# yuliangguo/OmniFusion

Measured on AMD Instinct MI355X. Metric: panoramas/sec at 512x1024 ERP, N=18 256^2 patches; equi2pers+pers2equi GB/s vs HBM peak, higher is better.
Workload: dtype f16x3 (fp16 hi/lo pairs, fp32 accumulate: fp32-class); 1 GPU; cfg2/cfg4 shard: 8 panoramas/GPU/step, 512x1024 ERP, fov 80, nrows 4 (18 patches); full single-pass spherical_fusion forward (confidence=True) at patch size 128 — the only size the reference network exists at (SURVEY 0.1); random-init weights (seed 42); inputs resident in HBM; resample pair at 18x256^2 reported in roofline_resample; per_gpu_batch=8, global_batch=8, parallelism=image-sharded x1, execution=3 forwards in flight per GPU on 3 streams (spherical_fusion.pipelined)

## Files before the change

### omnifusion_amd/csrc/omni_conv_up2_taps.hip

```cpp
#include <stdint.h>
#include "omni_conv_sh_common.h"

namespace {

struct TapsArgs {
    const void* src;
    const void* wt;
    const float* bias;
    void* dst;
    int M, Hl, Cout, act;
};

constexpr int TAP_BYTES = 32 * 256;

__device__ __forceinline__ void wait_taps_in_flight(int n)
{
    if (n >= 16) wait_vm<16>();
    else if (n == 14) wait_vm<14>();
    else if (n == 12) wait_vm<12>();
    else if (n == 10) wait_vm<10>();
    else if (n == 8) wait_vm<8>();
    else if (n == 6) wait_vm<6>();
    else if (n == 4) wait_vm<4>();
    else if (n == 2) wait_vm<2>();
    else wait_vm<0>();
}

template <int WL, int ROWS, int HALO>
__global__ __launch_bounds__(256, 1) void up2_taps_fused_kernel(TapsArgs a)
{
    static_assert((WL == 32 && ROWS == 8 && HALO == 1) || (WL == 16 && ROWS == 16 && HALO == 0), "bands of 8 rows of 32-wide maps, or whole 16 x 16 maps");
    constexpr int SROWS = ROWS + 2 * HALO, P = SROWS * WL, NF = P / 32, NFW = (NF + 3) / 4;
    constexpr int W_BYTES = 9 * TAP_BYTES, CH_BYTES = P * 128, ROW_BYTES = WL * 128;
    static_assert(P % 32 == 0 && ROWS * WL == 256, "whole fragments; one (column, channel quad) thread per eight rows");
    __shared__ __attribute__((aligned(1024))) unsigned char lds[W_BYTES + 2 * CH_BYTES];
    static_assert(sizeof(lds) <= 160 * 1024, "one block per CU");

    const int t = threadIdx.x, lane = t & 63;
    const int wave = __builtin_amdgcn_readfirstlane(t >> 6);
    const int ntn = a.Cout >> 5, nb = a.Hl / ROWS;
    int bid = blockIdx.x;
    const int tile_n = bid % ntn; bid /= ntn;
    const int band = bid % nb; const int m = bid / nb;
    const int r0 = band * ROWS, col0 = tile_n * 32, sbase = r0 - HALO;
    const int Hl = a.Hl;

    auto frag = [&](int fi) { const int f = wave + 4 * fi; return f < NF ? f : wave + 4; };
    h8v xh[NFW][4], xl[NFW][4];
#pragma unroll
    for (int fi = 0; fi < NFW; ++fi) {
        const int f = frag(fi);
        {
            const int p = f * 32 + (lane & 31), sr = p / WL, cx = p - sr * WL;
            const int row = min(max(sbase + sr, 0), Hl - 1);
            const unsigned char* sp = (const unsigned char*)a.src + ((size_t)(m * Hl + row) * WL + cx) * 256 + (lane >> 5) * 16;
#pragma unroll
            for (int kc = 0; kc < 4; ++kc) {
                xh[fi][kc] = *reinterpret_cast<const h8v*>(sp + (kc >> 1) * 128 + (kc & 1) * 32);
                xl[fi][kc] = *reinterpret_cast<const h8v*>(sp + (kc >> 1) * 128 + 64 + (kc & 1) * 32);
            }
        }
    }
    {
        const rsrc_t rsw = make_rsrc(a.wt, (size_t)9 * a.Cout * 256);
#pragma unroll
        for (int tp = 0; tp < 9; ++tp)
#pragma unroll
            for (int k = 0; k < 2; ++k) {
                const int i = wave + 4 * k, row = 4 * i + (lane >> 4), piece = (lane & 15) ^ (row & 15);
                dma16(rsw, lds + tp * TAP_BYTES + i * 1024, ((tp * a.Cout + col0 + row) * 16 + piece) * 16, 0);
            }
    }
    const int wfo = (lane & 31) * 256 + (((lane >> 5) ^ (lane & 15)) * 16);

    const int quad = t & 7, j = (t >> 3) & (WL - 1);
    const int ib = WL == 32 ? 0 : 8 * (wave >> 1);
    int coff[3];
#pragma unroll
    for (int c = 0; c < 3; ++c) {
        const int col = min(max(j - 1 + c, 0), WL - 1);
        coff[c] = col * 128 + ((quad ^ ((col >> 1) & 3)) * 16);
    }
    float hx[4], lx[4];
    hx[0] = j > 0 ? 0.75f : 0.0f;      lx[0] = j > 0 ? 0.25f : 0.0f;
    hx[1] = j > 0 ? 0.25f : 1.0f;      lx[1] = j > 0 ? 0.75f : 0.0f;
    hx[2] = 0.75f;                     lx[2] = 0.25f;
    hx[3] = j < WL - 1 ? 0.25f : 0.0f; lx[3] = j < WL - 1 ? 0.75f : 0.0f;

    f4v out[8][2][2];
#pragma unroll
    for (int it = 0; it < 8; ++it)
#pragma unroll
        for (int ab = 0; ab < 4; ++ab) out[it][ab >> 1][ab & 1] = (f4v)(0.0f);

    wait_taps_in_flight(16);
    __builtin_amdgcn_s_barrier();
    asm volatile("" ::: "memory");

    auto tap = [&]<int tp>() {
        constexpr int ky = tp / 3, kx = tp - 3 * ky;
        unsigned char* chunk = lds + W_BYTES + (tp & 1) * CH_BYTES;
        {
            const unsigned char* wb = lds + tp * TAP_BYTES;
            h8v wh[4], wl[4];
#pragma unroll
            for (int kc = 0; kc < 4; ++kc) {
                const int K = 8 * (kc >> 1) + 2 * (kc & 1);
                wh[kc] = *reinterpret_cast<const h8v*>(wb + (wfo ^ (K * 16)));
                wl[kc] = *reinterpret_cast<const h8v*>(wb + (wfo ^ ((K + 4) * 16)));
            }
#pragma unroll
            for (int fi = 0; fi < NFW; ++fi) {
                const int f = frag(fi);
                {
                    f16v acc = (f16v)(0.0f), acc1 = (f16v)(0.0f);
#pragma unroll
                    for (int kc = 0; kc < 4; ++kc) {
                        acc  = __builtin_amdgcn_mfma_f32_32x32x16_f16(wh[kc], xh[fi][kc], acc, 0, 0, 0);
                        acc1 = __builtin_amdgcn_mfma_f32_32x32x16_f16(wl[kc], xh[fi][kc], acc1, 0, 0, 0);
                        acc1 = __builtin_amdgcn_mfma_f32_32x32x16_f16(wh[kc], xl[fi][kc], acc1, 0, 0, 0);
                    }
                    const int px = f * 32 + (lane & 31);
                    unsigned char* cp = chunk + px * 128;
                    const int sw = (px >> 1) & 3;
#pragma unroll
                    for (int q = 0; q < 4; ++q) {
                        f4v v;
#pragma unroll
                        for (int e = 0; e < 4; ++e) v[e] = acc_join<false>(acc1[4 * q + e], acc[4 * q + e]);
                        *reinterpret_cast<f4v*>(cp + (((2 * q + (lane >> 5)) ^ sw) * 16)) = v;
                    }
                }
                __builtin_amdgcn_sched_barrier(0);
            }
        }
        if (tp < 8) wait_taps_in_flight(2 * (7 - tp));
        wait_lds_reads();
        __builtin_amdgcn_s_barrier();
        asm volatile("" ::: "memory");
#pragma unroll
        for (int it = 0; it < 8; ++it) {
            const int i = r0 + ib + it;
            float hy[4], ly[4];
            const bool top = it == 0 && i == 0, bot = it == 7 && i == Hl - 1;
            hy[0] = top ? 0.0f : 0.75f; ly[0] = top ? 0.0f : 0.25f;
            hy[1] = top ? 1.0f : 0.25f; ly[1] = top ? 0.0f : 0.75f;
            hy[2] = 0.75f;              ly[2] = 0.25f;
            hy[3] = bot ? 0.0f : 0.25f; ly[3] = bot ? 0.0f : 0.75f;
            f4v v[3][3];
#pragma unroll
            for (int r = 0; r < 3; ++r) {
                if (r < (ky >> 1) || r > ((ky + 1) >> 1) + 1) continue;
                const unsigned char* rp = chunk + (min(max(i - 1 + r, 0), Hl - 1) - sbase) * ROW_BYTES;
#pragma unroll
                for (int c = 0; c < 3; ++c) {
                    if (c < (kx >> 1) || c > ((kx + 1) >> 1) + 1) continue;
                    v[r][c] = *reinterpret_cast<const f4v*>(rp + coff[c]);
                }
            }
#pragma unroll
            for (int ay = 0; ay < 2; ++ay)
#pragma unroll
                for (int bx = 0; bx < 2; ++bx) {
                    const int uy = ay + ky, ux = bx + kx, r = uy >> 1, c = ux >> 1;
                    const float w00 = hy[uy] * hx[ux], w01 = hy[uy] * lx[ux], w10 = ly[uy] * hx[ux], w11 = ly[uy] * lx[ux];
                    f4v o = out[it][ay][bx];
#pragma unroll
                    for (int e = 0; e < 4; ++e)
                        o[e] = fmaf(w11, v[r + 1][c + 1][e], fmaf(w10, v[r + 1][c][e], fmaf(w01, v[r][c + 1][e], fmaf(w00, v[r][c][e], o[e]))));
                    asm volatile("" : "+v"(o));
                    out[it][ay][bx] = o;
                }
            __builtin_amdgcn_sched_barrier(0);
        }
    };
    tap.template operator()<0>(); tap.template operator()<1>(); tap.template operator()<2>();
    tap.template operator()<3>(); tap.template operator()<4>(); tap.template operator()<5>();
    tap.template operator()<6>(); tap.template operator()<7>(); tap.template operator()<8>();

    f4v bv = (f4v)(0.0f);
    if (a.bias) bv = *reinterpret_cast<const f4v*>(a.bias + col0 + quad * 4);
    const int Ho = 2 * Hl, Wo = 2 * WL;
#pragma unroll
    for (int it = 0; it < 8; ++it)
#pragma unroll
        for (int ay = 0; ay < 2; ++ay)
#pragma unroll
            for (int bx = 0; bx < 2; ++bx) {
                f4v o = out[it][ay][bx] + bv;
                if (a.act == OMNI_ACT_RELU) { o.x = fmaxf(o.x, 0.f); o.y = fmaxf(o.y, 0.f); o.z = fmaxf(o.z, 0.f); o.w = fmaxf(o.w, 0.f); }
                const int oy = 2 * (r0 + ib + it) + ay, ox = 2 * j + bx;
                act_store4<true>(a.dst, (((size_t)m * Ho + oy) * Wo + ox) * a.Cout + col0 + quad * 4, o);
            }
}

}

OMNI_SH_OVERFLOW_ACCESSOR(omni_sh_overflow_up2_taps)

extern "C" int omni_conv3x3_up2_taps_sh_f16x3(const void* src, const void* wt16t, const float* bias, void* dst, int fmt,
                                              int M, int Hl, int Wl, int C, int Cout, int act, omni_stream_t stream)
{
    if (!src || !wt16t || !dst) OMNI_FAIL(OMNI_ERR_INVALID, "omni_conv3x3_up2_taps_sh: null pointer");
    if (M <= 0 || Hl <= 0 || Wl <= 0 || C <= 0 || C % 32 || Cout <= 0 || Cout % 32) OMNI_FAIL(OMNI_ERR_INVALID, "omni_conv3x3_up2_taps_sh: bad shape (channels must be multiples of 32)");
    if ((uintptr_t)src % 16 || (uintptr_t)wt16t % 16 || (uintptr_t)bias % 16 || (uintptr_t)dst % 16) OMNI_FAIL(OMNI_ERR_INVALID, "omni_conv3x3_up2_taps_sh: tensors must be 16-byte aligned");
    const bool bands = Wl == 32 && Hl % 8 == 0, image = Wl == 16 && Hl == 16;
    if ((fmt & ~4) != 1 || C != 64 || Cout != 64 || !(bands || image) || (act != OMNI_ACT_NONE && act != OMNI_ACT_RELU))
        OMNI_FAIL(OMNI_ERR_UNSUPPORTED, "omni_conv3x3_up2_taps_sh: serves f16x3 with an SH result, 64 -> 64 channels, Wl = 32 with Hl % 8 == 0 or 16 x 16 maps, no activation or ReLU");
    if ((long long)M * Hl * Wl * 4 >= (1ll << 31)) OMNI_FAIL(OMNI_ERR_UNSUPPORTED, "omni_conv3x3_up2_taps_sh: tensor too large for 32-bit indices");
    TapsArgs a;
    a.src = src; a.wt = wt16t; a.bias = bias; a.dst = dst; a.M = M; a.Hl = Hl; a.Cout = Cout; a.act = act;
    const unsigned ntn = (unsigned)(Cout / 32);
    if (bands) hipLaunchKernelGGL((up2_taps_fused_kernel<32, 8, 1>), dim3((unsigned)M * (unsigned)(Hl / 8) * ntn), dim3(256), 0, (hipStream_t)stream, a);
    else       hipLaunchKernelGGL((up2_taps_fused_kernel<16, 16, 0>), dim3((unsigned)M * ntn), dim3(256), 0, (hipStream_t)stream, a);
    OMNI_HIP(hipGetLastError());
    return OMNI_OK;
}
```

### omnifusion_amd/isa.py

```python
import os
import re
import subprocess
import sys
import tempfile

LLVM = os.environ.get("OMNI_LLVM_BIN", "/opt/rocm/lib/llvm/bin")
TARGET = "hipv4-amdgcn-amd-amdhsa--gfx950"
FORBIDDEN = re.compile(r"\bv_pk_(mul|add|fma)_f32\b")
COUNTED = ("e2p_box_kernel", "p2e_lds_kernel", "p2e_walk_kernel", "e2p_ref_kernel")
HOT = ("conv_sh_kernel", "conv3x3_halo_sh_kernel", "conv3x3_up2_g1_kernel", "stem_f16x3_pc_kernel", "heads_kernel", "maxpool_kernel",
       "layernorm512_kernel", "attention_kernel", "upsample_sh8_kernel", "halo2_sh_kernel")
HOST_ONLY = ("omni_png.o", "omni_geometry.o")


def _device_object(obj, tmp):
    fat = os.path.join(tmp, "fat.bin")
    co = os.path.join(tmp, "dev.co")
    r = subprocess.run([os.path.join(LLVM, "llvm-objcopy"), "--dump-section", f".hip_fatbin={fat}", obj, os.path.join(tmp, "copy.o")],
                       stderr=subprocess.DEVNULL)
    if r.returncode != 0 or not os.path.exists(fat) or os.path.getsize(fat) == 0:
        return None
    subprocess.check_call([os.path.join(LLVM, "clang-offload-bundler"), "--unbundle", "--type=o", f"--input={fat}",
                           f"--targets={TARGET}", f"--output={co}"])
    return co


def disassemble(obj):
    with tempfile.TemporaryDirectory() as tmp:
        co = _device_object(obj, tmp)
        if co is None:
            return ""
        return subprocess.check_output([os.path.join(LLVM, "llvm-objdump"), "-d", "--mcpu=gfx950", co]).decode()


def kernel_meta(obj):
    with tempfile.TemporaryDirectory() as tmp:
        co = _device_object(obj, tmp)
        if co is None:
            return []
        txt = subprocess.check_output([os.path.join(LLVM, "llvm-readelf"), "--notes", co]).decode()
    out, cur = [], None
    keys = {".vgpr_count": "vgpr", ".agpr_count": "agpr", ".sgpr_count": "sgpr", ".group_segment_fixed_size": "lds",
            ".private_segment_fixed_size": "scratch", ".vgpr_spill_count": "vgpr_spill", ".sgpr_spill_count": "sgpr_spill",
            ".name": "name"}
    for line in txt.splitlines():
        m = re.match(r"^  - \.(\w+):\s*(\S+)\s*$", line)
        if m:
            cur = {}
            out.append(cur)
            line = "    ." + m.group(1) + ": " + m.group(2)
        m = re.match(r"^    (\.\w+):\s*(\S+)\s*$", line)
        if m and cur is not None and m.group(1) in keys:
            v = m.group(2)
            cur[keys[m.group(1)]] = v if m.group(1) == ".name" else int(v)
    return [k for k in out if "name" in k]


def demangle(names):
    try:
        p = subprocess.run([os.path.join(LLVM, "llvm-cxxfilt")], input="\n".join(names).encode(), stdout=subprocess.PIPE, check=True)
        return p.stdout.decode().splitlines()
    except Exception:
        return list(names)


def objects():
    from . import build as b
    return [s[:-4] + ".o" for s in b.sources()]


def check(objs=None):
    bad = []
    found = {c: 0 for c in COUNTED + HOT}
    full = objs is None
    for obj in objs or objects():
        base = os.path.basename(obj)
        if not os.path.exists(obj):
            bad.append(f"{base}: object missing (build first)")
            continue
        asm = disassemble(obj)
        if not asm.strip():
            if base not in HOST_ONLY:
                bad.append(f"{base}: no gfx950 device code could be extracted (not in HOST_ONLY): the ISA rules were NOT checked")
            continue
        cur = "?"
        for line in asm.splitlines():
            if line.endswith(">:"):
                cur = line.split("<", 1)[1][:-2]
            elif FORBIDDEN.search(line):
                bad.append(f"{base}: packed-fp32 instruction in {cur}: {line.strip()[:80]}")
                break
        for k in kernel_meta(obj):
            for c in COUNTED + HOT:
                if c in k["name"]:
                    found[c] += 1
            if any(c in k["name"] for c in COUNTED):
                if k.get("scratch", 0) or k.get("vgpr_spill", 0):
                    bad.append(f"{base}: {k['name']} uses scratch {k.get('scratch')} B / spills {k.get('vgpr_spill')} VGPR "
                               f"{k.get('sgpr_spill')} SGPR — its hand-counted s_waitcnt vmcnt(N) would be off")
            elif any(c in k["name"] for c in HOT):
                if k.get("scratch", 0) or k.get("vgpr_spill", 0):
                    bad.append(f"{base}: {k['name']} (a kernel with >= 1 % of the bench's GPU time) uses scratch {k.get('scratch')} B / "
                               f"spills {k.get('vgpr_spill')} VGPR")
    if full:
        for c, n in found.items():
            if n == 0:
                bad.append(f"guarded kernel `{c}` was not found in any code object's metadata: the scratch rule for it was NOT checked")
    return bad


def table(objs=None):
    rows = []
    for obj in objs or objects():
        meta = kernel_meta(obj)
        for k, nm in zip(meta, demangle([k["name"] for k in meta])):
            nm = nm.replace("(anonymous namespace)::", "")
            nm = re.sub(r"\(.*$", "", nm)
            rows.append((os.path.basename(obj), nm, k.get("vgpr", 0), k.get("agpr", 0), k.get("sgpr", 0), k.get("lds", 0), k.get("scratch", 0)))
    return rows


if __name__ == "__main__":
    if "--check" in sys.argv:
        v = check()
        for line in v:
            print("ISA CHECK FAILED:", line)
        print("isa check:", "FAILED" if v else "ok (no v_pk_*_f32; counted-wait and hot kernels without scratch; every guarded kernel found)")
        sys.exit(1 if v else 0)
    print(f"{'object':22s} {'vgpr':>4s} {'agpr':>4s} {'sgpr':>4s} {'lds':>6s} {'scr':>4s}  kernel")
    for o, nm, v, a, s, l, sc in table():
        print(f"{o:22s} {v:4d} {a:4d} {s:4d} {l:6d} {sc:4d}  {nm[:150]}")
```

Before: 4363 panoramas/s.

## Separate bilinear upsample into vertical then horizontal passes in up2 taps kernel

Reorders the 3x3 taps column-major so that, for each kx, the three ky taps accumulate a vertical-only interpolation into per-row registers. After the third ky tap, the kernel applies the horizontal interpolation by exchanging the vertically interpolated values through LDS with neighbouring columns. This replaces the full 2D bilinear gather per tap (up to 9 LDS loads and 4 weights each) with cheaper separable 1D passes that reuse row loads along a sliding window. The price is extra LDS stores and barriers for the horizontal exchange and more live registers. The kernel is also added to the ISA scratch-check list.

Result: faster. 4430 panoramas/s (median of 6 runs) (+1.5%).

```diff
diff --git a/omnifusion_amd/csrc/omni_conv_up2_taps.hip b/omnifusion_amd/csrc/omni_conv_up2_taps.hip
--- a/omnifusion_amd/csrc/omni_conv_up2_taps.hip
+++ b/omnifusion_amd/csrc/omni_conv_up2_taps.hip
@@ -26,6 +26,8 @@
     else wait_vm<0>();
 }
 
+__host__ __device__ constexpr int tap_at(int s) { return 3 * (s % 3) + s / 3; }
+
 template <int WL, int ROWS, int HALO>
 __global__ __launch_bounds__(256, 1) void up2_taps_fused_kernel(TapsArgs a)
 {
@@ -64,12 +66,14 @@
     {
         const rsrc_t rsw = make_rsrc(a.wt, (size_t)9 * a.Cout * 256);
 #pragma unroll
-        for (int tp = 0; tp < 9; ++tp)
+        for (int s = 0; s < 9; ++s) {
+            const int tp = tap_at(s);
 #pragma unroll
             for (int k = 0; k < 2; ++k) {
                 const int i = wave + 4 * k, row = 4 * i + (lane >> 4), piece = (lane & 15) ^ (row & 15);
                 dma16(rsw, lds + tp * TAP_BYTES + i * 1024, ((tp * a.Cout + col0 + row) * 16 + piece) * 16, 0);
             }
+        }
     }
     const int wfo = (lane & 31) * 256 + (((lane >> 5) ^ (lane & 15)) * 16);
 
@@ -87,19 +91,20 @@
     hx[2] = 0.75f;                     lx[2] = 0.25f;
     hx[3] = j < WL - 1 ? 0.25f : 0.0f; lx[3] = j < WL - 1 ? 0.75f : 0.0f;
 
+    const bool top = r0 + ib == 0, bot = r0 + ib + 7 == Hl - 1;
+    const float hy0[4] = {top ? 0.0f : 0.75f, top ? 1.0f : 0.25f, 0.75f, 0.25f}, ly0[4] = {top ? 0.0f : 0.25f, top ? 0.0f : 0.75f, 0.25f, 0.75f};
+    const float hy7 = bot ? 0.0f : 0.25f, ly7 = bot ? 0.0f : 0.75f;
+
     f4v out[8][2][2];
-#pragma unroll
-    for (int it = 0; it < 8; ++it)
-#pragma unroll
-        for (int ab = 0; ab < 4; ++ab) out[it][ab >> 1][ab & 1] = (f4v)(0.0f);
+    f4v S[8][2];
 
     wait_taps_in_flight(16);
     __builtin_amdgcn_s_barrier();
     asm volatile("" ::: "memory");
 
-    auto tap = [&]<int tp>() {
-        constexpr int ky = tp / 3, kx = tp - 3 * ky;
-        unsigned char* chunk = lds + W_BYTES + (tp & 1) * CH_BYTES;
+    auto tap = [&]<int s>() {
+        constexpr int tp = tap_at(s), ky = tp / 3, kx = tp - 3 * ky;
+        unsigned char* chunk = lds + W_BYTES + (s & 1) * CH_BYTES;
         {
             const unsigned char* wb = lds + tp * TAP_BYTES;
             h8v wh[4], wl[4];
@@ -134,44 +139,73 @@
                 __builtin_amdgcn_sched_barrier(0);
             }
         }
-        if (tp < 8) wait_taps_in_flight(2 * (7 - tp));
+        if (s < 8) wait_taps_in_flight(2 * (7 - s));
         wait_lds_reads();
         __builtin_amdgcn_s_barrier();
         asm volatile("" ::: "memory");
-#pragma unroll
-        for (int it = 0; it < 8; ++it) {
-            const int i = r0 + ib + it;
-            float hy[4], ly[4];
-            const bool top = it == 0 && i == 0, bot = it == 7 && i == Hl - 1;
-            hy[0] = top ? 0.0f : 0.75f; ly[0] = top ? 0.0f : 0.25f;
-            hy[1] = top ? 1.0f : 0.25f; ly[1] = top ? 0.0f : 0.75f;
-            hy[2] = 0.75f;              ly[2] = 0.25f;
-            hy[3] = bot ? 0.0f : 0.25f; ly[3] = bot ? 0.0f : 0.75f;
-            f4v v[3][3];
-#pragma unroll
-            for (int r = 0; r < 3; ++r) {
-                if (r < (ky >> 1) || r > ((ky + 1) >> 1) + 1) continue;
-                const unsigned char* rp = chunk + (min(max(i - 1 + r, 0), Hl - 1) - sbase) * ROW_BYTES;
-#pragma unroll
-                for (int c = 0; c < 3; ++c) {
-                    if (c < (kx >> 1) || c > ((kx + 1) >> 1) + 1) continue;
-                    v[r][c] = *reinterpret_cast<const f4v*>(rp + coff[c]);
-                }
-            }
-#pragma unroll
-            for (int ay = 0; ay < 2; ++ay)
-#pragma unroll
-                for (int bx = 0; bx < 2; ++bx) {
-                    const int uy = ay + ky, ux = bx + kx, r = uy >> 1, c = ux >> 1;
-                    const float w00 = hy[uy] * hx[ux], w01 = hy[uy] * lx[ux], w10 = ly[uy] * hx[ux], w11 = ly[uy] * lx[ux];
-                    f4v o = out[it][ay][bx];
+        {
+            constexpr int klo = ky >> 1, khi = 8 + ((ky + 1) >> 1);
+            f4v R[10];
+#pragma unroll
+            for (int k = klo; k <= khi; ++k)
+                R[k] = *reinterpret_cast<const f4v*>(chunk + (min(max(r0 + ib - 1 + k, 0), Hl - 1) - sbase) * ROW_BYTES + coff[1]);
+#pragma unroll
+            for (int it = 0; it < 8; ++it)
+#pragma unroll
+                for (int ay = 0; ay < 2; ++ay) {
+                    const int uy = ay + ky, r = uy >> 1;
+                    const float h = it == 0 ? hy0[uy] : it == 7 && uy == 3 ? hy7 : (uy & 1) ? 0.25f : 0.75f;
+                    const float l = it == 0 ? ly0[uy] : it == 7 && uy == 3 ? ly7 : (uy & 1) ? 0.75f : 0.25f;
+                    f4v v;
+                    if constexpr (ky != 0) v = S[it][ay];
 #pragma unroll
                     for (int e = 0; e < 4; ++e)
-                        o[e] = fmaf(w11, v[r + 1][c + 1][e], fmaf(w10, v[r + 1][c][e], fmaf(w01, v[r][c + 1][e], fmaf(w00, v[r][c][e], o[e]))));
-                    asm volatile("" : "+v"(o));
-                    out[it][ay][bx] = o;
+                        if constexpr (ky == 0) v[e] = fmaf(l, R[it + r + 1][e], h * R[it + r][e]);
+                        else v[e] = fmaf(l, R[it + r + 1][e], fmaf(h, R[it + r][e], v[e]));
+                    asm volatile("" : "+v"(v));
+                    S[it][ay] = v;
                 }
             __builtin_amdgcn_sched_barrier(0);
+        }
+        if constexpr (ky == 2) {
+            unsigned char* other = lds + W_BYTES + ((s & 1) ^ 1) * CH_BYTES;
+            auto horizontal = [&]<int ay>(const unsigned char* buf) {
+#pragma unroll
+                for (int it = 0; it < 8; ++it) {
+                    const unsigned char* rp = buf + (ib + it) * ROW_BYTES;
+                    const f4v own = S[it][ay];
+                    f4v left = own, right = own;
+                    if (kx <= 1) left = *reinterpret_cast<const f4v*>(rp + coff[0]);
+                    if (kx >= 1) right = *reinterpret_cast<const f4v*>(rp + coff[2]);
+#pragma unroll
+                    for (int bx = 0; bx < 2; ++bx) {
+                        const int ux = bx + kx, c = ux >> 1;
+                        const f4v va = c == 0 ? left : own, vb = c == 0 ? own : right;
+                        f4v o;
+                        if constexpr (kx != 0) o = out[it][ay][bx];
+#pragma unroll
+                        for (int e = 0; e < 4; ++e)
+                            if constexpr (kx == 0) o[e] = fmaf(lx[ux], vb[e], hx[ux] * va[e]);
+                            else o[e] = fmaf(lx[ux], vb[e], fmaf(hx[ux], va[e], o[e]));
+                        asm volatile("" : "+v"(o));
+                        out[it][ay][bx] = o;
+                    }
+                }
+                __builtin_amdgcn_sched_barrier(0);
+            };
+#pragma unroll
+            for (int it = 0; it < 8; ++it) *reinterpret_cast<f4v*>(other + (ib + it) * ROW_BYTES + coff[1]) = S[it][0];
+            wait_lds_reads();
+            __builtin_amdgcn_s_barrier();
+            asm volatile("" ::: "memory");
+#pragma unroll
+            for (int it = 0; it < 8; ++it) *reinterpret_cast<f4v*>(chunk + (ib + it) * ROW_BYTES + coff[1]) = S[it][1];
+            __builtin_amdgcn_sched_barrier(0);
+            horizontal.template operator()<0>(other);
+            wait_lds_reads();
+            __builtin_amdgcn_s_barrier();
+            asm volatile("" ::: "memory");
+            horizontal.template operator()<1>(chunk);
         }
     };
     tap.template operator()<0>(); tap.template operator()<1>(); tap.template operator()<2>();
diff --git a/omnifusion_amd/isa.py b/omnifusion_amd/isa.py
--- a/omnifusion_amd/isa.py
+++ b/omnifusion_amd/isa.py
@@ -7,7 +7,7 @@
 LLVM = os.environ.get("OMNI_LLVM_BIN", "/opt/rocm/lib/llvm/bin")
 TARGET = "hipv4-amdgcn-amd-amdhsa--gfx950"
 FORBIDDEN = re.compile(r"\bv_pk_(mul|add|fma)_f32\b")
-COUNTED = ("e2p_box_kernel", "p2e_lds_kernel", "p2e_walk_kernel", "e2p_ref_kernel")
+COUNTED = ("e2p_box_kernel", "p2e_lds_kernel", "p2e_walk_kernel", "e2p_ref_kernel", "up2_taps_fused_kernel")
 HOT = ("conv_sh_kernel", "conv3x3_halo_sh_kernel", "conv3x3_up2_g1_kernel", "stem_f16x3_pc_kernel", "heads_kernel", "maxpool_kernel",
        "layernorm512_kernel", "attention_kernel", "upsample_sh8_kernel", "halo2_sh_kernel")
 HOST_ONLY = ("omni_png.o", "omni_geometry.o")
```
